# lionl1106/Clip-Neural-image-conpression

Hardware: AMD Instinct MI355X
Metric: images/sec @256px 50-step DDIM, batch=8/GPU (higher is better)
Workload: dtype bf16; 1 GPU; 256px base=128 ch_mult=(1, 2, 2) 50-step DDIM (eta=0), batch=8/GPU, key-seeded synthetic weights (out.* x0.1), synthetic z / x_T; global_batch=8, parallelism=dp1 (independent batches, no collective in the loop), graph=hipGraph, one replay per step, steps_in_flight=1

## Files before the change

clip-neural-image-conpression_amd/csrc/ccn_conv_pr.hip:

```cpp
#include "ccn_device.h"
#include <cstdio>
#include <cstdlib>
#include <cstring>
#include <vector>
#include <algorithm>

namespace ccn {

namespace {

#define CCN_FDIV(x, m, d) ((m) ? (int)__umulhi((unsigned)(x), (m)) : (int)(x))

template <int TH_> struct PrLdsT {
    static constexpr int HROWS = TH_ + 2, HPITCH = 34;
    static constexpr int A_BYTES = HROWS * HPITCH * 128;
    static constexpr int SP = 272;
    static constexpr int STG_BYTES = TH_ * 32 * SP;
    static constexpr int CHS_BYTES = 4 * 128 * 2 * 4;
    static constexpr int TOTAL = 2 * A_BYTES + STG_BYTES + CHS_BYTES;
};
typedef PrLdsT<8> PrLds;
static_assert(PrLds::TOTAL <= 160 * 1024, "LDS budget");

}

template <int NTAPS, int D, int MODE, int TH = 8, int GS = 0, bool P4 = false>
__global__ __launch_bounds__(512) void conv_pr_kernel(const ConvArgs a, const int grid_tiles)
{
    static_assert(TH == 8 || (TH == 4 && NTAPS == 9), "4-row tiles: 3x3 stride-1 form only");
    static_assert(!P4 || (NTAPS == 4 && MODE != 2), "plane passes of 2x2 taps: the 4-tap consumers, no split-K");
    constexpr bool RES = MODE == 1;
    constexpr bool RR = MODE != 0;
    typedef __bf16 T;
    constexpr int MF = 4, NF = 2;
    constexpr int BN = 128;
    constexpr int HROWS = TH + 2;
    constexpr int OSC = (NTAPS == 4 && !P4) ? 2 : 1, NPARC = (NTAPS == 4 && !P4) ? 4 : 1;
    constexpr int EPC = 8, CKE = 64;
    constexpr int NSTEP = NTAPS * 4;
    constexpr bool S2 = NTAPS == 2;
    constexpr int NPASS = S2 ? 5 : (P4 ? 4 : 1);
    constexpr int IS = (S2 || P4) ? 2 : 1;
    static_assert(NSTEP % D == 0, "the register ring must wrap at the chunk boundary");
    using L = PrLdsT<TH>;
    constexpr int HPITCH = L::HPITCH;
    extern __shared__ __attribute__((aligned(16))) unsigned char smem[];
    unsigned char* const stg = smem + 2 * L::A_BYTES;

    const int tid = threadIdx.x, lane = tid & 63, wave = tid >> 6;
    const int r = lane & 31, h = lane >> 5;

    const int grid = (int)gridDim.x;
    const int vb = (grid & 7) == 0 ? ((int)blockIdx.x & 7) * (grid >> 3) + ((int)blockIdx.x >> 3) : (int)blockIdx.x;
    const int ntiles = grid_tiles;
    const int my_tiles = (ntiles - vb + grid - 1) / grid;
    auto vt = [&](int ti) __attribute__((always_inline)) { return vb + ti * grid; };
    const int ks = (MODE == 2 && a.ksplit == 2) ? 2 : 1;
    const unsigned xcc_id = MODE == 2 ? (unsigned)__builtin_amdgcn_s_getreg((3 << 11) | 20) : 0u;
    const int nck = a.nchunk / ks;
    const int ktotal = my_tiles * nck;
    auto vt_tile = [&](int v) __attribute__((always_inline)) { return ks == 2 ? (v >> 1) : v; };
    auto vt_kh = [&](int v) __attribute__((always_inline)) { return ks == 2 ? (v & 1) : 0; };

    const unsigned char* const inb = (const unsigned char*)a.in;
    constexpr bool gstat = GS == 1;
    static_assert(GS != 1 || (NTAPS == 9 && MODE != 2), "in-kernel statistics: 3x3 stride-1 layers without split-K");
    const bool gn = NTAPS == 9 && GS != 2 && !CCN_DBG_BIT(a, 32);
    constexpr unsigned OOB = 0x7FFFFFF0u;
    auto raw_barrier = [&]() __attribute__((always_inline)) {
        asm volatile("s_waitcnt lgkmcnt(0)" ::: "memory");
        __builtin_amdgcn_s_barrier();
        asm volatile("" ::: "memory");
    };
    auto stamp = [&](int slot) __attribute__((always_inline)) {
        if (CCN_STAMPS_PTR(a) && lane == 0 && (wave == 0 || wave == 4))
            CCN_STAMPS_PTR(a)[((size_t)blockIdx.x * 2 + (wave == 0 ? 0 : 1)) * 8 + slot] = __builtin_amdgcn_s_memrealtime();
    };
    [[maybe_unused]] unsigned long long t_bar = 0, t_a = 0, t_b = 0, t_w = 0, t_r = 0;
    const unsigned long long t_begin = CCN_STAMPS_PTR(a) ? __builtin_amdgcn_s_memtime() : 0;
    auto timed_barrier = [&]() __attribute__((always_inline)) {
        if (CCN_STAMPS_PTR(a)) { const unsigned long long t0 = __builtin_amdgcn_s_memtime(); raw_barrier(); t_bar += __builtin_amdgcn_s_memtime() - t0; }
        else raw_barrier();
    };
    auto stamp_cycles = [&]() __attribute__((always_inline)) {
        if (CCN_STAMPS_PTR(a) && lane == 0 && (wave == 0 || wave == 4)) {
            unsigned long long* st = CCN_STAMPS_PTR(a) + ((size_t)blockIdx.x * 2 + (wave == 0 ? 0 : 1)) * 8;
            st[3] = t_bar; st[4] = __builtin_amdgcn_s_memtime() - t_begin; st[5] = t_a; st[6] = t_b; st[7] = t_r;
        }
    };
    stamp(0);

    const int etid = tid & 255, ew = wave & 3;
    const int o16 = etid & 15, pr = etid >> 4;
    unsigned char* const outb = (unsigned char*)a.out;
    const unsigned char* const resb = (const unsigned char*)a.res;
    const unsigned out_bytes = (unsigned)((size_t)a.B * a.Hout * a.Wout * a.Cout * sizeof(T));
    float* const chs = (float*)(stg + L::STG_BYTES) + ew * 256;
    constexpr int NQ = TH / 2;
    u32x4 rr[RR ? 2 : 1][4];
    f32x4 fb[2], fs[RES ? 1 : 2], ft[RES ? 1 : 2];
    int e_b = 0, e_ty = 0, e_tx = 0, e_nt = 0, e_par = 0, e_kh = 0, e_tile = 0;
    bool pd_on = false;
    int pd_b = 0, pd_slot = 0, pd_n0 = 0;
    unsigned char* const kpartb = (unsigned char*)a.kpart;
    unsigned e_base = 0;
    int e_rows = 0;
    unsigned e_m0 = OOB, e_m1 = OOB;
    auto item_off = [&](unsigned eb, int it) __attribute__((always_inline)) -> unsigned {
        const unsigned rmask = (it >> 1) < e_rows ? 0u : OOB;
        return (eb + (unsigned)(it >> 1) * (unsigned)(OSC * a.Wout * a.Cout * (int)sizeof(T)) + (unsigned)((it & 1) * 16) * (unsigned)(OSC * a.Cout * (int)sizeof(T)))
               | ((it & 1) ? e_m1 : e_m0) | rmask;
    };
    auto epi_setup = [&](int v) __attribute__((always_inline)) {
        const int tile = vt_tile(v);
        e_kh = vt_kh(v); e_tile = tile;
        const int t2 = CCN_FDIV(tile, a.fd_nt, a.n_nt);
        e_nt = tile - t2 * a.n_nt;
        e_par = t2 % NPARC;
        const int sp = t2 / NPARC;
        {
            const int row = CCN_FDIV(sp, a.fd_tx, a.n_tx);
            e_tx = sp - row * a.n_tx;
            e_b = CCN_FDIV(sp, a.fd_sp, a.n_tx * a.n_ty);
            e_ty = row - e_b * a.n_ty;
        }
        const int nb = e_nt * BN + o16 * 8;
        const bool nvalid = nb < a.Cout;
        e_base = (unsigned)(((e_b * a.Hout + e_ty * TH * OSC + (e_par >> 1)) * a.Wout + (e_tx * 32 + pr) * OSC + (e_par & 1)) * a.Cout + nb) * (unsigned)sizeof(T);
        e_rows = a.MH - e_ty * TH;
        e_m0 = (nvalid && e_tx * 32 + pr < a.MW) ? 0u : OOB;
        e_m1 = (nvalid && e_tx * 32 + pr + 16 < a.MW) ? 0u : OOB;
    };
    auto res_on = [&]() __attribute__((always_inline)) -> bool { return RES || (MODE == 2 && ks == 2 && e_kh == 1); };
    auto res_batch = [&](int q, u32x4* dst) __attribute__((always_inline)) {
        if constexpr (RR) {
            if (res_on()) {
                const auto srd = __builtin_amdgcn_make_buffer_rsrc((void*)((ks == 2 && e_kh == 1) ? kpartb : (resb ? resb : outb)), 0, out_bytes, 0x00020000);
                unsigned eb = e_base; asm volatile("" : "+v"(eb));
                if (ks == 2 && e_kh == 1) {
#pragma unroll
// ... 88 lines not shown
                if (live) {
#pragma unroll
                    for (int e = 0; e < 8; ++e) { s1[e] += x[e]; s2[e] = fmaf(x[e], x[e], s2[e]); }
                }
                asm volatile("" : "+v"(s1[0]), "+v"(s1[1]), "+v"(s1[2]), "+v"(s1[3]), "+v"(s1[4]), "+v"(s1[5]), "+v"(s1[6]), "+v"(s1[7]));
                asm volatile("" : "+v"(s2[0]), "+v"(s2[1]), "+v"(s2[2]), "+v"(s2[3]), "+v"(s2[4]), "+v"(s2[5]), "+v"(s2[6]), "+v"(s2[7]));
                __builtin_amdgcn_sched_barrier(0);
            }
            if constexpr (RR) { if (q + 2 < q1) res_batch(q + 2, rr[q & 1]); }
        }
        if (first) {
            asm volatile("s_waitcnt vmcnt(0)" ::: "memory");
            if (lane == 0) __hip_atomic_store(a.kflag + (size_t)e_tile * 4 + ew, xcc_id + 1u, __ATOMIC_RELAXED, __HIP_MEMORY_SCOPE_AGENT);
        }
        if (a.part && !first) {
#pragma unroll
            for (int s = 16; s < 64; s <<= 1)
#pragma unroll
                for (int e = 0; e < 8; ++e) { s1[e] += __shfl_xor(s1[e], s); s2[e] += __shfl_xor(s2[e], s); }
            if (lane < 16) {
#pragma unroll
                for (int e = 0; e < 8; ++e) { chs[(lane * 8 + e) * 2] = s1[e]; chs[(lane * 8 + e) * 2 + 1] = s2[e]; }
            }
            pd_on = true; pd_b = e_b; pd_n0 = e_nt * BN;
            pd_slot = ((e_ty * a.n_tx + e_tx) * NPARC + e_par) * a.n_nt + e_nt;
        }
    };
    auto combine = [&]() __attribute__((always_inline)) {
        if (!pd_on) return;
        pd_on = false;
        const float* const all = (const float*)(stg + L::STG_BYTES);
        const int n0 = pd_n0;
        if (n0 >= a.Cout) return;
        const int nend = min(n0 + BN, a.Cout);
        const int g1 = CCN_FDIV(nend - 1, a.fd_cpg, a.cpg);
        for (int g = CCN_FDIV(n0, a.fd_cpg, a.cpg) + ew; g <= g1; g += 4) {
            const int clo = max(g * a.cpg, n0), chi = min((g + 1) * a.cpg, nend);
            float t1 = 0.f, t2 = 0.f;
            const float* const wa = all + (lane >> 4) * 256;
            for (int c = clo + (lane & 15); c < chi; c += 16) {
                t1 += wa[(c - n0) * 2]; t2 += wa[(c - n0) * 2 + 1];
            }
#pragma unroll
            for (int m = 32; m >= 1; m >>= 1) { t1 += __shfl_xor(t1, m); t2 += __shfl_xor(t2, m); }
            if (lane == 0) part_store(a.part + (size_t)(pd_b * a.G + g) * a.nslot + pd_slot, t1, t2);
        }
    };

    const int ptid = tid & 255;
    const int ck = ptid & 7, pcol = ptid >> 3;
    const int xrow = pcol >> 1, xcol = 32 + (pcol & 1);
    const bool xthr = ptid < HROWS * 16;
    constexpr int AIT = HROWS + 1;
    u32x4 areg[AIT];
    GnCoef<T> gk;
    unsigned rowm = 0;
    bool colv = false, xv = false;
    int rq_ti = 0, rq_c = 0;
    GnCoef<T> gkn;
    int q_b = 0, q_iy0 = 0, q_ix0 = 0, q_c = 0;
    bool q_tv = false;
    float st_mean = 0.f, st_rstd = 1.f, qn_mean = 0.f, qn_rstd = 1.f;
    int st_b = -1;
    f32x4 qn_g[2], qn_bt[2];
    unsigned svmask = 0u;
    float2 sv[8];
    auto stats_issue = [&](int b) __attribute__((always_inline)) {
        const int g = lane >> 3, sub = lane & 7;
        const int cpg = a.gs_cpg, pnt = a.gs_nnt, nsp = a.gs_nsp;
        const int jlo = CCN_FDIV(g * cpg, a.fd_gsbn, a.gs_bn), jhi = CCN_FDIV((g + 1) * cpg - 1, a.fd_gsbn, a.gs_bn), nj = jhi - jlo + 1;
        const float2* const base = a.gs_part + (size_t)(b * 8 + g) * ((size_t)nsp * pnt) + jlo;
        int off[8];
        svmask = 0u;
#pragma unroll
        for (int u = 0; u < 8; ++u) {
            const int e = sub + 8 * u;
            const int jj = CCN_FDIV(e, a.fd_gsnsp, nsp), sp = e - jj * nsp;
            const bool ok = jj < nj;
            off[u] = ok ? sp * pnt + jj : 0;
            svmask |= ok ? (1u << u) : 0u;
        }
#pragma unroll
        for (int u = 0; u < 8; ++u) sv[u] = base[off[u]];
    };
    auto stats_reduce = [&]() __attribute__((always_inline)) {
        double s1 = 0.0, s2 = 0.0;
#pragma unroll
        for (int u = 0; u < 8; ++u) { const bool ok = (svmask >> u) & 1u; s1 += ok ? (double)sv[u].x : 0.0; s2 += ok ? (double)sv[u].y : 0.0; }
#pragma unroll
        for (int m = 1; m < 8; m <<= 1) { s1 += __shfl_xor(s1, m); s2 += __shfl_xor(s2, m); }
        const double mean = s1 * a.gs_inv_count;
        double var = s2 * a.gs_inv_count - mean * mean;
        if (var < 0.0) var = 0.0;
        st_mean = (float)mean;
        st_rstd = __builtin_amdgcn_rsqf((float)(var + 1e-5));
    };
    int q_cbs = 0; bool q_cv = false, q_cv_i = false;
    auto decode = [&]() __attribute__((always_inline)) -> bool {
        const int v = vt(rq_ti);
        if (rq_c == 0) {
            q_tv = rq_ti < my_tiles;
            const int tile = vt_tile(q_tv ? v : vt(0));
            const int sp = CCN_FDIV(tile, a.fd_ntp, a.n_nt * NPARC);
            const int row = CCN_FDIV(sp, a.fd_tx, a.n_tx);
            const int tx = sp - row * a.n_tx;
            q_b = CCN_FDIV(sp, a.fd_sp, a.n_tx * a.n_ty);
            const int ty = row - q_b * a.n_ty;
            q_iy0 = ty * TH - 1; q_ix0 = tx * 32 - 1;
        }
        q_c = vt_kh(v) * nck + rq_c;
        const int cb = (q_c / NPASS) * CKE + ck * EPC;
        q_cv = q_tv && cb < a.Cin;
        q_cbs = q_cv ? cb : 0;
        const bool fresh = gstat && rq_c == 0 && q_tv && q_b != st_b;
        if (++rq_c == nck) { rq_c = 0; ++rq_ti; }
        return fresh;
    };
    auto coef_loads = [&]() __attribute__((always_inline)) {
        if (gstat) {
            qn_g[0] = *(const f32x4*)(a.gs_gamma + q_cbs); qn_g[1] = *(const f32x4*)(a.gs_gamma + q_cbs + 4);
            qn_bt[0] = *(const f32x4*)(a.gs_beta + q_cbs); qn_bt[1] = *(const f32x4*)(a.gs_beta + q_cbs + 4);
        } else gkn.load(a.gn_ab + (size_t)q_b * a.Cin + q_cbs, gn && q_cv);
    };
    auto coef_sel = [&]() __attribute__((always_inline)) {
        if (gstat) {
            const int src = CCN_FDIV(q_cbs, a.fd_gscpg, a.gs_cpg) * 8;
            qn_mean = __shfl(st_mean, src); qn_rstd = __shfl(st_rstd, src);
        }
    };
    auto prep = [&]() __attribute__((always_inline)) {
        const bool fresh = decode();
        coef_loads();
        if (fresh) { stats_issue(q_b); stats_reduce(); st_b = q_b; }
        coef_sel();
    };
    auto adopt = [&]() __attribute__((always_inline)) {
        if (gstat) gk.from_raw(qn_g, qn_bt, qn_mean, qn_rstd, gn && q_cv_i);
        else gk = gkn;
    };
    auto issue_loads = [&](int r0 = 0, int r1 = TH + 2, bool with_x = true) __attribute__((always_inline)) {
        const int b = __builtin_amdgcn_readfirstlane(q_b), iy0 = __builtin_amdgcn_readfirstlane(q_iy0), ix0 = __builtin_amdgcn_readfirstlane(q_ix0);
        const int cc = __builtin_amdgcn_readfirstlane(q_c / NPASS);
        const int pass = q_c - cc * NPASS;
        const int py = S2 ? (pass <= 2 ? 1 : 0) : (P4 ? (pass < 2 ? 1 : 0) : 0);
        const int px = S2 ? ((pass <= 1 || pass == 3) ? 1 : 0) : (P4 ? ((pass & 1) ? 0 : 1) : 0);
        const int cb = cc * CKE + ck * EPC;
        const bool cv = q_tv && cb < a.Cin;
        q_cv_i = cv;
        const unsigned img_bytes = (unsigned)(a.Hin * a.Win * a.Cin) * (unsigned)sizeof(T);
        const unsigned coff = (unsigned)(((q_tv && cc * CKE < a.Cin) ? cc : 0) * CKE) * (unsigned)sizeof(T);
        const auto srd = __builtin_amdgcn_make_buffer_rsrc((void*)(inb + (size_t)b * img_bytes + coff), 0, img_bytes - coff, 0x00020000);
        const int rs = IS * a.Win * a.Cin * (int)sizeof(T);
        const int ixr = IS * (ix0 + pcol) + px;
        colv = cv && ixr >= 0 && ixr < a.Win;
        const unsigned cmask = colv ? 0u : OOB;
        const int base = ((IS * iy0 + py) * a.Win + ixr) * a.Cin * (int)sizeof(T) + ck * 16;
        const int first = IS * iy0 + py;
        const int r_lo = first < 0 ? (-first + IS - 1) / IS : 0;
        int r_hi = (a.Hin - first + IS - 1) / IS; r_hi = r_hi > HROWS ? HROWS : (r_hi < 0 ? 0 : r_hi);
        rowm = q_tv ? (((1u << r_hi) - 1u) & ~((1u << r_lo) - 1u)) : 0u;
#pragma unroll
        for (int i = 0; i < HROWS; ++i) {
            if (i < r0 || i >= r1) continue;
            areg[i] = __builtin_amdgcn_raw_buffer_load_b128(srd, (unsigned)(base + i * rs) | cmask, 0, 0);
        }
        {
            const int iyr = IS * (iy0 + xrow) + py, ixx = IS * (ix0 + xcol) + px;
            xv = xthr && cv && iyr >= 0 && iyr < a.Hin && ixx >= 0 && ixx < a.Win;
            const int off = (iyr * a.Win + ixx) * a.Cin * (int)sizeof(T) + ck * 16;
            if (with_x) areg[HROWS] = __builtin_amdgcn_raw_buffer_load_b128(srd, (unsigned)off | (xv ? 0u : OOB), 0, 0);
        }
    };
    auto issue = [&]() __attribute__((always_inline)) { issue_loads(); adopt(); };
    auto request = [&]() __attribute__((always_inline)) { prep(); issue(); };
    auto request_first = [&](int r0, int r1, bool with_x) __attribute__((always_inline)) {
        const bool fresh = decode();
        if (fresh) stats_issue(q_b);
        coef_loads();
        issue_loads(r0, r1, with_x);
        if (fresh) { stats_reduce(); st_b = q_b; }
        coef_sel();
        adopt();
    };
    auto dump = [&](int buf, int r0 = 0, int r1 = TH + 2, bool with_x = true) __attribute__((always_inline)) {
        unsigned char* const As = smem + buf * L::A_BYTES;
        int pc = pcol; asm volatile("" : "+v"(pc));
#pragma unroll
        for (int i = 0; i < AIT; ++i) {
            if (i < HROWS ? (i < r0 || i >= r1) : !with_x) continue;
            const int px = i < HROWS ? i * HPITCH + pc : (pc >> 1) * HPITCH + 32 + (pc & 1);
            const int sw = i < HROWS ? (NTAPS == 9 ? (pc >> 1) & 3 : (pc >> 1)) : 0;
            u32x4 v = areg[i];
            const bool ok = i < HROWS ? (((rowm >> i) & 1u) && colv) : xv;
            if (gn) {
                const u32x4 tr = gk.template apply<true>(v);
                v = u32x4{0u, 0u, 0u, 0u};
                if (ok) v = tr;
            }
            if (i < HROWS || xthr) *(u32x4*)(As + px * 128 + (((ck ^ sw) & 7) << 4)) = v;
            if ((i & 1) == 1) __builtin_amdgcn_sched_barrier(0);
        }
    };

    constexpr int HSPLIT = HROWS / 2;

    if (wave >= 4) {
        if (a.prod_first) __builtin_amdgcn_s_setprio(3);
        if (CCN_DBG_BIT(a, 128)) __builtin_amdgcn_s_setprio(1);
        if (CCN_DBG_BIT(a, 256)) __builtin_amdgcn_s_setprio(3);
        request_first(0, HSPLIT, true);
        dump(0, 0, HSPLIT, true);
        request();
        raw_barrier();
        stamp(1);
        int c = 0, ti = 0;
        for (int k = 0; k < ktotal; ++k) {
            unsigned long long t0 = CCN_STAMPS_PTR(a) ? __builtin_amdgcn_s_memtime() : 0;
            if (CCN_STAMPS_PTR(a)) {
                asm volatile("s_waitcnt vmcnt(0)" ::: "memory");
                const unsigned long long t1 = __builtin_amdgcn_s_memtime(); t_w += t1 - t0; t0 = t1;
            }
            if (k + 1 < ktotal) { prep(); dump((k + 1) & 1); }
            if (CCN_STAMPS_PTR(a)) { const unsigned long long t1 = __builtin_amdgcn_s_memtime(); t_a += t1 - t0; t0 = t1; }
            const bool epi = c == 0 && ti > 0;
            if (epi) epi_request(0, NQ);
            if (k + 1 < ktotal) issue();
            if (c == nck - 1) epi_setup(vt(ti));
            if (CCN_STAMPS_PTR(a)) { const unsigned long long t1 = __builtin_amdgcn_s_memtime(); t_r += t1 - t0; t0 = t1; }
            if (epi) epilogue(0, NQ);
            if (CCN_STAMPS_PTR(a)) t_b += __builtin_amdgcn_s_memtime() - t0;
            const bool early = k + 1 == ktotal && !(ks == 2 && e_kh == 1);
            if (early) epi_request(0, NQ);
            timed_barrier();
            combine();
            if (++c == nck) { c = 0; ++ti; }
        }
        if (ks == 2 && e_kh == 1) epi_request(0, NQ);
        epilogue(0, NQ);
        if (pd_on) {
            raw_barrier();
            combine();
        }
        stamp(2); stamp_cycles();
        return;
    }

    if (!CCN_DBG_BIT(a, 16)) __builtin_amdgcn_s_setprio(2);
    if constexpr (NTAPS == 9) {
        constexpr int NROW = HROWS, NSG = 2 * NROW;
        constexpr int NG = 6;
        constexpr int WIN = 6, PF = 4;
        static_assert((NG * NSG) % WIN == 0, "static window indexing");
        f32x16 acc[TH];
        const int n32 = a.Cout_pad / 32;
        constexpr unsigned COLB = 36 * 1024;
        const unsigned wtotal = (unsigned)((size_t)a.nchunk * n32 * COLB);
        const auto wsrd = __builtin_amdgcn_make_buffer_rsrc((void*)a.wfrag, 0, wtotal, 0x00020000);
        const unsigned lane16 = (unsigned)lane * 16u;
        auto wbase_of = [&](int tile, int chunk) __attribute__((always_inline)) -> unsigned {
            const int nt = tile - CCN_FDIV(tile, a.fd_nt, a.n_nt) * a.n_nt;
            return (unsigned)__builtin_amdgcn_readfirstlane((int)((unsigned)(chunk * n32 + nt * 4 + wave) * COLB));
        };
        const int px16 = lane & 15, g4 = lane >> 4;
        int b16x[3];
#pragma unroll
        for (int d = 0; d < 3; ++d) { const int hx = px16 + d; b16x[d] = hx * 128 + ((((g4 & 1) << 2) | ((g4 >> 1) ^ ((hx >> 1) & 3))) << 4); }
        u32x4 bq[2][3][2];
        {
            const unsigned wb = wbase_of(vt_tile(vt(0)), vt_kh(vt(0)) * nck);
#pragma unroll
            for (int f = 0; f < 6; ++f) bq[0][f >> 1][f & 1] = __builtin_amdgcn_raw_buffer_load_b128(wsrd, lane16, wb + f * 1024, 0);
        }
        const int stg_lane = px16 * L::SP + (wave * 32 + 4 * g4) * 2;
        if constexpr (HSPLIT < HROWS) {
            request_first(HSPLIT, HROWS, false);
            if (CCN_STAMPS_PTR(a)) {
                const unsigned long long r0 = CCN_STAMPS_PTR(a)[((size_t)blockIdx.x * 2) * 8];
                t_a = __builtin_amdgcn_s_memrealtime() - r0;
                asm volatile("s_waitcnt vmcnt(0)" ::: "memory");
                t_b = __builtin_amdgcn_s_memrealtime() - r0;
            }
            dump(0, HSPLIT, HROWS, false);
            if (CCN_STAMPS_PTR(a)) t_r = __builtin_amdgcn_s_memrealtime() - CCN_STAMPS_PTR(a)[((size_t)blockIdx.x * 2) * 8];
        }
        raw_barrier();
        stamp(1);
        int k = 0;
        const bool idle_w = ks == 1 && grid % a.n_nt == 0 &&
                            (vt_tile(vt(0)) - CCN_FDIV(vt_tile(vt(0)), a.fd_nt, a.n_nt) * a.n_nt) * BN + wave * 32 >= a.Cout;
        if (idle_w) { for (int kk = 0; kk < ktotal; ++kk) timed_barrier(); }
        else
        for (int ti = 0; ti < my_tiles; ++ti) {
            const int v = vt(ti), v_next = ti + 1 < my_tiles ? vt(ti + 1) : v;
            const int tile = vt_tile(v), c0 = vt_kh(v) * nck;
#pragma unroll
            for (int i = 0; i < TH; ++i)
#pragma unroll
                for (int q = 0; q < 16; ++q) acc[i][q] = 0.0f;
            for (int chunk = 0; chunk < nck; ++chunk, ++k) {
                const unsigned wb_cur = wbase_of(tile, c0 + chunk);
                const unsigned wb_nxt = chunk + 1 < nck ? wbase_of(tile, c0 + chunk + 1) : wbase_of(vt_tile(v_next), vt_kh(v_next) * nck);
                int bufoff = (k & 1) * L::A_BYTES; asm volatile("" : "+v"(bufoff));
                u32x4 rw[WIN];
                int ag = 0;
                auto rload = [&](int s_) __attribute__((always_inline)) {
                    const int g = s_ / NSG, hp = s_ % NSG;
                    if (hp == 0) ag = (bufoff + b16x[g >> 1]) ^ ((g & 1) << 5);
                    rw[s_ % WIN] = *(const u32x4*)(smem + ag + ((hp >> 1) * HPITCH + (hp & 1) * 16) * 128);
                };
                if (!CCN_DBG_BIT(a, 64)) {
#pragma unroll
                for (int s_ = 0; s_ < PF; ++s_) rload(s_);
#pragma unroll
                for (int s_ = 0; s_ < NG * NSG; ++s_) {
                    const int g = s_ / NSG, hh = (s_ % NSG) >> 1, p = s_ & 1;
                    __builtin_amdgcn_sched_barrier(0);
                    const bool wl = TH == 8 ? (p == 0 && hh >= 2 && hh <= 7) : (hh >= 1 && hh <= 3);
                    if (wl) {
                        const int f = TH == 8 ? hh - 2 : (hh - 1) * 2 + p;
                        const unsigned off = g + 1 < NG ? wb_cur + (unsigned)((g + 1) * 6 + f) * 1024u : wb_nxt + (unsigned)f * 1024u;
                        bq[(g + 1) & 1][f >> 1][f & 1] = __builtin_amdgcn_raw_buffer_load_b128(wsrd, lane16, off, 0);
                    }
                    if (s_ + PF < NG * NSG) rload(s_ + PF);
                    int nm = 0;
#pragma unroll
                    for (int q6 = 0; q6 < 6; ++q6) {
                        const int o = (s_ & 1) ? 5 - q6 : q6;
                        const int dy = o >> 1, c = o & 1;
                        const int i = hh - dy;
                        if (i >= 0 && i < TH) { mfma16q(acc[i], p * 2 + c, bq[g & 1][dy][c], rw[s_ % WIN]); ++nm; }
                    }
#pragma unroll
                    for (int m = 0; m < 6; ++m) {
                        if (m < nm) __builtin_amdgcn_sched_group_barrier(0x008, 1, 0);
                        if (m == 0) __builtin_amdgcn_sched_group_barrier(0x100, 1, 0);
                        if (m == 2 && wl) __builtin_amdgcn_sched_group_barrier(0x020, 1, 0);
// ... 156 lines not shown
    }
    if (gs == 2 && ntaps == 9) {
        if (th == 4) return mode == 1 ? (pr_fn_t)conv_pr_kernel<9, PR_D, 1, 4, 2> : (mode == 2 ? (pr_fn_t)conv_pr_kernel<9, PR_D, 2, 4, 2> : (pr_fn_t)conv_pr_kernel<9, PR_D, 0, 4, 2>);
        return mode == 1 ? (pr_fn_t)conv_pr_kernel<9, PR_D, 1, 8, 2> : (mode == 2 ? (pr_fn_t)conv_pr_kernel<9, PR_D, 2, 8, 2> : (pr_fn_t)conv_pr_kernel<9, PR_D, 0, 8, 2>);
    }
    if (ntaps == 9 && th == 4) return mode == 1 ? (pr_fn_t)conv_pr_kernel<9, PR_D, 1, 4> : (mode == 2 ? (pr_fn_t)conv_pr_kernel<9, PR_D, 2, 4> : (pr_fn_t)conv_pr_kernel<9, PR_D, 0, 4>);
    if (ntaps == 9) return mode == 1 ? (pr_fn_t)conv_pr_kernel<9, PR_D, 1> : (mode == 2 ? (pr_fn_t)conv_pr_kernel<9, PR_D, 2> : (pr_fn_t)conv_pr_kernel<9, PR_D, 0>);
    if (ntaps == 2) return mode == 1 ? (pr_fn_t)conv_pr_kernel<2, 8, 1> : (mode == 2 ? (pr_fn_t)conv_pr_kernel<2, 8, 2> : (pr_fn_t)conv_pr_kernel<2, 8, 0>);
    return mode == 1 ? (pr_fn_t)conv_pr_kernel<4, 8, 1> : (mode == 2 ? (pr_fn_t)conv_pr_kernel<4, 8, 2> : (pr_fn_t)conv_pr_kernel<4, 8, 0>);
}

bool conv_pr_supported(int kind, int bn, int th)
{
    return bn == 128 && (((kind == KIND_C3S1 || kind == KIND_CT4 || kind == KIND_C3S2) && th == 8) || (kind == KIND_C3S1 && th == 4));
}

static int g_cus = 0;
hipError_t conv_pr_prepare()
{
    hipError_t e = hipSuccess;
    for (int ntaps : {2, 4, 9, 16})
        for (int mode = 0; mode < 3; ++mode) {
            if (ntaps == 16 && mode == 2) continue;
            e = hipFuncSetAttribute((const void*)pick_pr(ntaps, mode), hipFuncAttributeMaxDynamicSharedMemorySize, (int)PrLds::TOTAL);
            if (e != hipSuccess) return e;
        }
    for (int mode = 0; mode < 3; ++mode) {
        e = hipFuncSetAttribute((const void*)pick_pr(9, mode, 4), hipFuncAttributeMaxDynamicSharedMemorySize, (int)PrLdsT<4>::TOTAL);
        if (e != hipSuccess) return e;
    }
    for (int gs = 1; gs <= 2; ++gs)
        for (int mode = 0; mode < 3; ++mode) {
            if (gs == 1 && mode == 2) continue;
            e = hipFuncSetAttribute((const void*)pick_pr(9, mode, 8, gs), hipFuncAttributeMaxDynamicSharedMemorySize, (int)PrLds::TOTAL);
            if (e != hipSuccess) return e;
            e = hipFuncSetAttribute((const void*)pick_pr(9, mode, 4, gs), hipFuncAttributeMaxDynamicSharedMemorySize, (int)PrLdsT<4>::TOTAL);
            if (e != hipSuccess) return e;
        }
    int dev = 0;
    e = hipGetDevice(&dev);
    if (e != hipSuccess) return e;
    hipDeviceProp_t prop;
    e = hipGetDeviceProperties(&prop, dev);
    if (e != hipSuccess) return e;
    g_cus = prop.multiProcessorCount;
    return hipSuccess;
}

static unsigned long long* g_stamps = nullptr;
static unsigned g_stamp_grid = 0;
extern "C" int ccn_internal_dump_stamps_pr(const char* path)
{
    if (!g_stamps || !g_stamp_grid) return 1;
    std::vector<unsigned long long> hbuf((size_t)g_stamp_grid * 16);
    if (hipMemcpy(hbuf.data(), g_stamps, hbuf.size() * 8, hipMemcpyDeviceToHost) != hipSuccess) return 2;
    FILE* f = fopen(path, "w");
    if (!f) return 3;
    for (unsigned b = 0; b < g_stamp_grid; ++b)
        for (int k = 0; k < 16; ++k) fprintf(f, "%llu%c", hbuf[(size_t)b * 16 + k], k == 15 ? '\n' : ' ');
    fclose(f);
    return 0;
}

hipError_t launch_conv_pr(int dtype, const ConvArgs& a, hipStream_t s)
{
    const bool c3 = a.ntaps == 9 && a.npar == 1 && a.OS == 1, ct = a.ntaps == 4 && a.npar == 4 && a.OS == 2;
    const bool s2 = a.ntaps == 2 && a.npar == 1 && a.OS == 1 && !a.gn_ab && (a.nchunk % 5) == 0;
    const bool p4 = a.ntaps == 16 && a.npar == 1 && a.OS == 1 && (a.nchunk % 4) == 0 && a.ksplit != 2;
    if ((ct || s2 || p4) && (a.gn_ab || a.gs_part)) return hipErrorInvalidValue;
    if (dtype != 1 || !a.wfrag || !(c3 || ct || s2 || p4) || !(a.th == 8 || (a.th == 4 && c3)) || (a.Cout_pad & 127) || a.nchunk < 2 || a.fin_counter || (a.res && a.film)) return hipErrorInvalidValue;
    const int ks = a.ksplit == 2 ? 2 : 1;
    if (ks == 2 && (!a.kpart || !a.kflag || (a.nchunk & 1) || (s2 && (a.nchunk / 2) % 5) || a.res)) return hipErrorInvalidValue;
    const int ntiles = a.B * a.n_ty * a.n_tx * a.npar * a.n_nt * ks;
    static const int cap = diag_env("CCN_PR_GRID") ? atoi(diag_env("CCN_PR_GRID")) : 0;
    int grid = cap > 0 ? cap : (g_cus > 0 ? g_cus : 256);
    if (grid > ntiles) grid = ntiles;
    if (ks == 2) { grid &= ~15; if (grid < 16) return hipErrorInvalidValue; }
    ConvArgs d = a;
    {
        auto magic = [](long dv) -> unsigned { return dv <= 1 ? 0u : (unsigned)((0x100000000ull + (unsigned long long)dv - 1) / (unsigned long long)dv); };
        const long dmax = std::max<long>(std::max<long>((long)a.n_nt * a.npar, (long)a.n_tx * a.n_ty), std::max<long>(a.cpg, a.gs_cpg));
        if ((unsigned long long)std::max<long>(ntiles, 8192) * (unsigned long long)dmax >= 0x100000000ull) return hipErrorInvalidValue;
        d.fd_nt = magic(a.n_nt); d.fd_ntp = magic((long)a.n_nt * a.npar); d.fd_tx = magic(a.n_tx); d.fd_sp = magic((long)a.n_tx * a.n_ty);
        d.fd_cpg = magic(a.cpg); d.fd_gscpg = magic(a.gs_cpg);
        d.fd_gsbn = magic(a.gs_bn); d.fd_gsnsp = magic(a.gs_nsp);
    }
    d.prod_first = (a.nchunk <= 2 && c3) ? 1 : 0;
    static const char* env = diag_env("CCN_STAMPS");
    if (env && (unsigned)atoi(env) == (unsigned)ntiles && (!strchr(env, ':') || atoi(strchr(env, ':') + 1) == a.ntaps)) {
        if (!g_stamps) { if (hipMalloc((void**)&g_stamps, (size_t)1024 * 24 * 8) != hipSuccess) return hipErrorOutOfMemory; }
        g_stamp_grid = (unsigned)grid;
        d.stamps = g_stamps;
    } else d.stamps = nullptr;
    if (a.gs_part && !(c3 && ks == 1)) return hipErrorInvalidValue;
    hipLaunchKernelGGL(pick_pr(a.ntaps, a.res ? 1 : (ks == 2 ? 2 : 0), a.th, a.gs_part ? 1 : (a.gn_ab ? 0 : 2)), dim3((unsigned)grid), dim3(512),
                       a.th == 4 ? PrLdsT<4>::TOTAL : PrLds::TOTAL, s, d, ntiles);
    return hipGetLastError();
}

}
```

clip-neural-image-conpression_amd/csrc/ccn_kernels.hip:

```cpp
#include "ccn_conv_tile.h"

namespace ccn {

__host__ __device__ constexpr int cmax(int a, int b) { return a > b ? a : b; }

template <int AK, int IS> struct HaloGeom {
    static constexpr int HOFF = AK == A_NHWC ? 1 : 0;
    static constexpr int ROWS = AK == A_NHWC ? (IS == 1 ? 6 : 10) : 4;
    static constexpr int PITCH = AK == A_NHWC ? (IS == 1 ? 34 : 66) : 32;
    static constexpr int BYTES = ROWS * PITCH * 128;
};
template <int AK, int IS, int BN> struct LdsGeom {
    static constexpr int A_BYTES = HaloGeom<AK, IS>::BYTES;
    static constexpr int B_BYTES = BN * 128;
    static constexpr int TOTAL = EpiLds<4, BN, 4>::total(A_BYTES + 2 * B_BYTES);
};

template <typename T, int AK, int IS, int EPI, int WM, int WN, int MF, int NF>
__global__ __launch_bounds__(256) void conv_igemm_kernel(const ConvArgs a)
{
    static_assert(WM * WN == 4 && WM * MF == 4, "4 waves, 4 M-fragments of 32 pixels (TH=4 rows of TW=32)");
    constexpr int BN = WN * NF * 32;
    constexpr int EPC = Vec16<T>::EPC;
    constexpr int CKE = 8 * EPC;
// ... 632 lines not shown
    const int per = (HW + nslot - 1) / nslot;
    const int p0 = slot * per, p1 = min(HW, p0 + per);
    const int nsub = 256 / G;
    const int g = tid % G, sub = tid / G;
    float s1 = 0.f, s2 = 0.f;
    if (sub < nsub)
        for (int p = p0 + sub; p < p1; p += nsub) {
            const T* row = x + ((size_t)b * HW + p) * C + g * cpg;
            for (int j = 0; j < cpg; ++j) { const float v = (float)row[j]; s1 += v; s2 = fmaf(v, v, s2); }
        }
    sh[tid * 2] = s1; sh[tid * 2 + 1] = s2;
    __syncthreads();
    if (tid < G) {
        float t1 = 0.f, t2 = 0.f;
        for (int q = 0; q < nsub; ++q) { t1 += sh[(q * G + tid) * 2]; t2 += sh[(q * G + tid) * 2 + 1]; }
        part[(size_t)(b * G + tid) * nslot + slot] = make_float2(t1, t2);
    }
}
hipError_t launch_gn_partials(int dtype, const void* x, float2* part, int B, int HW, int C, int cpg, int G, int nslot, hipStream_t s)
{
    if (G > 256) return hipErrorInvalidValue;
    if (dtype == 0) hipLaunchKernelGGL(gn_partials_kernel<float>, dim3(nslot, B), dim3(256), 0, s, (const float*)x, part, HW, C, cpg, G, nslot);
    else hipLaunchKernelGGL(gn_partials_kernel<__bf16>, dim3(nslot, B), dim3(256), 0, s, (const __bf16*)x, part, HW, C, cpg, G, nslot);
    return hipGetLastError();
}

template <typename TI>
__global__ void temb_kernel(const TI* __restrict__ t, float* __restrict__ out, int n, int dim)
{
    const int half = dim / 2;
    const int idx = blockIdx.x * blockDim.x + threadIdx.x;
    if (idx >= n * dim) return;
    const int row = idx / dim, i = idx - row * dim;
    float v = 0.0f;
    if (i < 2 * half) {
        const int fi = i < half ? i : i - half;
        const float f = expf(__fdiv_rn(__fmul_rn(-9.210340371976184f, (float)fi), (float)half));
        const float arg = __fmul_rn((float)t[row], f);
        v = i < half ? cosf(arg) : sinf(arg);
    }
    out[idx] = v;
}
hipError_t launch_temb_i64(const int64_t* t, float* out, int n, int dim, hipStream_t s)
{
    hipLaunchKernelGGL(temb_kernel<int64_t>, dim3((n * dim + 255) / 256), dim3(256), 0, s, t, out, n, dim);
    return hipGetLastError();
}
hipError_t launch_temb_i32(const int32_t* t, float* out, int n, int dim, hipStream_t s)
{
    hipLaunchKernelGGL(temb_kernel<int32_t>, dim3((n * dim + 255) / 256), dim3(256), 0, s, t, out, n, dim);
    return hipGetLastError();
}

__global__ __launch_bounds__(256) void linear_kernel(const float* __restrict__ xa, const float* __restrict__ xb, int a_div, int b_mod,
                                                      const float* __restrict__ W, const float* __restrict__ bias, float* __restrict__ y,
                                                      int R, int K, int N, int act_silu)
{
    const int lane = threadIdx.x & 63, wave = threadIdx.x >> 6;
    const int n = blockIdx.x * 4 + wave;
    if (n >= N) return;
    const int r0 = blockIdx.y * 16, r1 = min(R, r0 + 16);
    const float* wrow = W + (size_t)n * K;
    for (int rr = r0; rr < r1; ++rr) {
        const float* pa = xa + (size_t)(rr / a_div) * K;
        const float* pb = xb ? xb + (size_t)(rr % b_mod) * K : nullptr;
        float acc = 0.f;
        for (int k = lane; k < K; k += 64) {
            float xv = pa[k];
            if (pb) xv += pb[k];
            acc = fmaf(xv, wrow[k], acc);
        }
#pragma unroll
        for (int s = 32; s >= 1; s >>= 1) acc += __shfl_xor(acc, s);
        if (lane == 0) {
            float v = acc + (bias ? bias[n] : 0.f);
            if (act_silu) v = v / (1.0f + expf(-v));
            y[(size_t)rr * N + n] = v;
        }
    }
}
hipError_t launch_linear(const float* xa, const float* xb, int a_div, int b_mod, const float* W, const float* b, float* y,
                         int R, int K, int N, int act_silu, hipStream_t s)
{
    hipLaunchKernelGGL(linear_kernel, dim3((N + 3) / 4, (R + 15) / 16), dim3(256), 0, s, xa, xb, a_div, b_mod, W, b, y, R, K, N, act_silu);
    return hipGetLastError();
}

__global__ void ddim_step_kernel(float* __restrict__ x, const float* __restrict__ eps, const float* __restrict__ noise,
                                 float c0, float c1, float c2, float c3, float sigma, int64_t n)
{
    for (int64_t i = (int64_t)blockIdx.x * blockDim.x + threadIdx.x; i < n; i += (int64_t)gridDim.x * blockDim.x) {
        const float e = eps[i];
        float x0 = __fdiv_rn(__fsub_rn(x[i], __fmul_rn(c0, e)), c1);
        x0 = fminf(fmaxf(x0, -1.0f), 1.0f);
        float xn = __fadd_rn(__fmul_rn(c2, x0), __fmul_rn(c3, e));
        if (noise) xn = __fadd_rn(xn, __fmul_rn(sigma, noise[i]));
        x[i] = xn;
    }
}
hipError_t launch_ddim_step(float* x, const float* eps, const float* noise, float c0, float c1, float c2, float c3, float sigma,
                            int64_t n, hipStream_t s)
{
    const int grid = (int)((n + 255) / 256 < 4096 ? (n + 255) / 256 : 4096);
    hipLaunchKernelGGL(ddim_step_kernel, dim3(grid > 0 ? grid : 1), dim3(256), 0, s, x, eps, noise, c0, c1, c2, c3, sigma, n);
    return hipGetLastError();
}

__global__ void q_sample_kernel(float* __restrict__ out, const float* __restrict__ x0, const float* __restrict__ noise,
                                const float* __restrict__ a, const float* __restrict__ sg, int64_t per)
{
    const int b = blockIdx.y;
    const float ca = a[b], cs = sg[b];
    const size_t base = (size_t)b * per;
    for (int64_t i = (int64_t)blockIdx.x * blockDim.x + threadIdx.x; i < per; i += (int64_t)gridDim.x * blockDim.x)
        out[base + i] = __fadd_rn(__fmul_rn(ca, x0[base + i]), __fmul_rn(cs, noise[base + i]));
}
hipError_t launch_q_sample(float* out, const float* x0, const float* noise, const float* a, const float* sg, int B, int64_t per,
                           hipStream_t s)
{
    const int gx = (int)((per + 255) / 256 < 1024 ? (per + 255) / 256 : 1024);
    hipLaunchKernelGGL(q_sample_kernel, dim3(gx > 0 ? gx : 1, B), dim3(256), 0, s, out, x0, noise, a, sg, per);
    return hipGetLastError();
}

__global__ void predict_x0_kernel(float* __restrict__ out, const float* __restrict__ xt, const float* __restrict__ eps,
                                  const float* __restrict__ a, const float* __restrict__ sg, int64_t per)
{
    const int b = blockIdx.y;
    const float ca = a[b], cs = sg[b];
    const size_t base = (size_t)b * per;
    for (int64_t i = (int64_t)blockIdx.x * blockDim.x + threadIdx.x; i < per; i += (int64_t)gridDim.x * blockDim.x)
        out[base + i] = __fdiv_rn(__fsub_rn(xt[base + i], __fmul_rn(cs, eps[base + i])), ca);
}
hipError_t launch_predict_x0(float* out, const float* xt, const float* eps, const float* a, const float* sg, int B, int64_t per,
                             hipStream_t s)
{
    const int gx = (int)((per + 255) / 256 < 1024 ? (per + 255) / 256 : 1024);
// ... 58 lines not shown
```

Before: 83.83 images/sec.

## Double-buffer plane-pass register loads and register-tile the linear kernel

For the 2- and 4-tap conv forms, the register staging ring gets two sets so that loads for chunk k+2 are in flight while chunk k+1 is dumped to LDS. This hides global load latency at the cost of more VGPRs. Separately, the small linear kernel now keeps the weight row in registers, processes four rows per batch with interleaved shuffles, and covers 32 rows per block. The stamp instrumentation is widened to record the extra counters.

Result: no change. 83.33 images/sec (-0.6%).

```diff
diff --git a/clip-neural-image-conpression_amd/csrc/ccn_conv_pr.hip b/clip-neural-image-conpression_amd/csrc/ccn_conv_pr.hip
--- a/clip-neural-image-conpression_amd/csrc/ccn_conv_pr.hip
+++ b/clip-neural-image-conpression_amd/csrc/ccn_conv_pr.hip
@@ -4,12 +4,17 @@
 #include <cstring>
 #include <vector>
 #include <algorithm>
+#include <type_traits>
 
 namespace ccn {
 
 namespace {
 
 #define CCN_FDIV(x, m, d) ((m) ? (int)__umulhi((unsigned)(x), (m)) : (int)(x))
+
+#ifndef CCN_PR_PLANE_DEPTH
+#define CCN_PR_PLANE_DEPTH 2
+#endif
 
 template <int TH_> struct PrLdsT {
     static constexpr int HROWS = TH_ + 2, HPITCH = 34;
@@ -42,6 +47,7 @@
     constexpr int NPASS = S2 ? 5 : (P4 ? 4 : 1);
     constexpr int IS = (S2 || P4) ? 2 : 1;
     static_assert(NSTEP % D == 0, "the register ring must wrap at the chunk boundary");
+    constexpr int DEPTH = (CCN_PR_PLANE_DEPTH == 2 && (NTAPS == 2 || NTAPS == 4)) ? 2 : 1;
     using L = PrLdsT<TH>;
     constexpr int HPITCH = L::HPITCH;
     extern __shared__ __attribute__((aligned(16))) unsigned char smem[];
@@ -74,7 +80,7 @@
     };
     auto stamp = [&](int slot) __attribute__((always_inline)) {
         if (CCN_STAMPS_PTR(a) && lane == 0 && (wave == 0 || wave == 4))
-            CCN_STAMPS_PTR(a)[((size_t)blockIdx.x * 2 + (wave == 0 ? 0 : 1)) * 8 + slot] = __builtin_amdgcn_s_memrealtime();
+            CCN_STAMPS_PTR(a)[((size_t)blockIdx.x * 3 + (wave == 0 ? 0 : 1)) * 8 + slot] = __builtin_amdgcn_s_memrealtime();
     };
     [[maybe_unused]] unsigned long long t_bar = 0, t_a = 0, t_b = 0, t_w = 0, t_r = 0;
     const unsigned long long t_begin = CCN_STAMPS_PTR(a) ? __builtin_amdgcn_s_memtime() : 0;
@@ -84,8 +90,14 @@
     };
     auto stamp_cycles = [&]() __attribute__((always_inline)) {
         if (CCN_STAMPS_PTR(a) && lane == 0 && (wave == 0 || wave == 4)) {
-            unsigned long long* st = CCN_STAMPS_PTR(a) + ((size_t)blockIdx.x * 2 + (wave == 0 ? 0 : 1)) * 8;
+            unsigned long long* st = CCN_STAMPS_PTR(a) + ((size_t)blockIdx.x * 3 + (wave == 0 ? 0 : 1)) * 8;
             st[3] = t_bar; st[4] = __builtin_amdgcn_s_memtime() - t_begin; st[5] = t_a; st[6] = t_b; st[7] = t_r;
+            if (wave == 4) {
+                unsigned long long* sx = CCN_STAMPS_PTR(a) + ((size_t)blockIdx.x * 3 + 2) * 8;
+                sx[0] = t_w; sx[1] = (unsigned long long)ktotal; sx[2] = (unsigned long long)DEPTH;
+#pragma unroll
+                for (int i = 3; i < 8; ++i) sx[i] = 0;
+            }
         }
     };
     stamp(0);
@@ -280,10 +292,10 @@
     const int xrow = pcol >> 1, xcol = 32 + (pcol & 1);
     const bool xthr = ptid < HROWS * 16;
     constexpr int AIT = HROWS + 1;
-    u32x4 areg[AIT];
+    u32x4 areg[DEPTH][AIT];
     GnCoef<T> gk;
-    unsigned rowm = 0;
-    bool colv = false, xv = false;
+    unsigned rowm[DEPTH] = {};
+    bool colv[DEPTH] = {}, xv[DEPTH] = {};
     int rq_ti = 0, rq_c = 0;
     GnCoef<T> gkn;
     int q_b = 0, q_iy0 = 0, q_ix0 = 0, q_c = 0;
@@ -366,7 +378,7 @@
         if (gstat) gk.from_raw(qn_g, qn_bt, qn_mean, qn_rstd, gn && q_cv_i);
         else gk = gkn;
     };
-    auto issue_loads = [&](int r0 = 0, int r1 = TH + 2, bool with_x = true) __attribute__((always_inline)) {
+    auto issue_loads = [&](int r0 = 0, int r1 = TH + 2, bool with_x = true, int set = 0) __attribute__((always_inline)) {
         const int b = __builtin_amdgcn_readfirstlane(q_b), iy0 = __builtin_amdgcn_readfirstlane(q_iy0), ix0 = __builtin_amdgcn_readfirstlane(q_ix0);
         const int cc = __builtin_amdgcn_readfirstlane(q_c / NPASS);
         const int pass = q_c - cc * NPASS;
@@ -380,27 +392,28 @@
         const auto srd = __builtin_amdgcn_make_buffer_rsrc((void*)(inb + (size_t)b * img_bytes + coff), 0, img_bytes - coff, 0x00020000);
         const int rs = IS * a.Win * a.Cin * (int)sizeof(T);
         const int ixr = IS * (ix0 + pcol) + px;
-        colv = cv && ixr >= 0 && ixr < a.Win;
-        const unsigned cmask = colv ? 0u : OOB;
+        colv[set] = cv && ixr >= 0 && ixr < a.Win;
+        const unsigned cmask = colv[set] ? 0u : OOB;
         const int base = ((IS * iy0 + py) * a.Win + ixr) * a.Cin * (int)sizeof(T) + ck * 16;
         const int first = IS * iy0 + py;
         const int r_lo = first < 0 ? (-first + IS - 1) / IS : 0;
         int r_hi = (a.Hin - first + IS - 1) / IS; r_hi = r_hi > HROWS ? HROWS : (r_hi < 0 ? 0 : r_hi);
-        rowm = q_tv ? (((1u << r_hi) - 1u) & ~((1u << r_lo) - 1u)) : 0u;
+        rowm[set] = q_tv ? (((1u << r_hi) - 1u) & ~((1u << r_lo) - 1u)) : 0u;
 #pragma unroll
         for (int i = 0; i < HROWS; ++i) {
             if (i < r0 || i >= r1) continue;
-            areg[i] = __builtin_amdgcn_raw_buffer_load_b128(srd, (unsigned)(base + i * rs) | cmask, 0, 0);
+            areg[set][i] = __builtin_amdgcn_raw_buffer_load_b128(srd, (unsigned)(base + i * rs) | cmask, 0, 0);
         }
         {
             const int iyr = IS * (iy0 + xrow) + py, ixx = IS * (ix0 + xcol) + px;
-            xv = xthr && cv && iyr >= 0 && iyr < a.Hin && ixx >= 0 && ixx < a.Win;
+            xv[set] = xthr && cv && iyr >= 0 && iyr < a.Hin && ixx >= 0 && ixx < a.Win;
             const int off = (iyr * a.Win + ixx) * a.Cin * (int)sizeof(T) + ck * 16;
-            if (with_x) areg[HROWS] = __builtin_amdgcn_raw_buffer_load_b128(srd, (unsigned)off | (xv ? 0u : OOB), 0, 0);
+            if (with_x) areg[set][HROWS] = __builtin_amdgcn_raw_buffer_load_b128(srd, (unsigned)off | (xv[set] ? 0u : OOB), 0, 0);
         }
     };
     auto issue = [&]() __attribute__((always_inline)) { issue_loads(); adopt(); };
     auto request = [&]() __attribute__((always_inline)) { prep(); issue(); };
+    auto request_set = [&](int set) __attribute__((always_inline)) { prep(); issue_loads(0, TH + 2, true, set); adopt(); };
     auto request_first = [&](int r0, int r1, bool with_x) __attribute__((always_inline)) {
         const bool fresh = decode();
         if (fresh) stats_issue(q_b);
@@ -410,7 +423,7 @@
         coef_sel();
         adopt();
     };
-    auto dump = [&](int buf, int r0 = 0, int r1 = TH + 2, bool with_x = true) __attribute__((always_inline)) {
+    auto dump = [&](int buf, int r0 = 0, int r1 = TH + 2, bool with_x = true, int set = 0) __attribute__((always_inline)) {
         unsigned char* const As = smem + buf * L::A_BYTES;
         int pc = pcol; asm volatile("" : "+v"(pc));
 #pragma unroll
@@ -418,8 +431,8 @@
             if (i < HROWS ? (i < r0 || i >= r1) : !with_x) continue;
             const int px = i < HROWS ? i * HPITCH + pc : (pc >> 1) * HPITCH + 32 + (pc & 1);
             const int sw = i < HROWS ? (NTAPS == 9 ? (pc >> 1) & 3 : (pc >> 1)) : 0;
-            u32x4 v = areg[i];
-            const bool ok = i < HROWS ? (((rowm >> i) & 1u) && colv) : xv;
+            u32x4 v = areg[set][i];
+            const bool ok = i < HROWS ? (((rowm[set] >> i) & 1u) && colv[set]) : xv[set];
             if (gn) {
                 const u32x4 tr = gk.template apply<true>(v);
                 v = u32x4{0u, 0u, 0u, 0u};
@@ -438,10 +451,50 @@
         if (CCN_DBG_BIT(a, 256)) __builtin_amdgcn_s_setprio(3);
         request_first(0, HSPLIT, true);
         dump(0, 0, HSPLIT, true);
-        request();
+        if constexpr (DEPTH == 2) {
+            request_set(1);
+            __builtin_amdgcn_sched_barrier(0);
+            request_set(0);
+        } else request();
         raw_barrier();
         stamp(1);
         int c = 0, ti = 0;
+        if constexpr (DEPTH == 2) {
+            auto iter2 = [&](const int k, auto set_c) __attribute__((always_inline)) {
+                constexpr int set = decltype(set_c)::value;
+                unsigned long long t0 = CCN_STAMPS_PTR(a) ? __builtin_amdgcn_s_memtime() : 0;
+                if (CCN_STAMPS_PTR(a)) {
+                    asm volatile("s_waitcnt vmcnt(%0)" :: "n"(AIT) : "memory");
+                    const unsigned long long t1 = __builtin_amdgcn_s_memtime(); t_w += t1 - t0; t0 = t1;
+                }
+                if (set == 1 || k + 1 < ktotal) dump((k + 1) & 1, 0, TH + 2, true, set);
+                if (CCN_STAMPS_PTR(a)) { const unsigned long long t1 = __builtin_amdgcn_s_memtime(); t_a += t1 - t0; t0 = t1; }
+                const bool epi = c == 0 && ti > 0;
+                if (epi) epi_request(0, NQ);
+                if (c == nck - 1) epi_setup(vt(ti));
+                if (CCN_STAMPS_PTR(a)) { const unsigned long long t1 = __builtin_amdgcn_s_memtime(); t_r += t1 - t0; t0 = t1; }
+                if (epi) epilogue(0, NQ);
+                if (CCN_STAMPS_PTR(a)) { const unsigned long long t1 = __builtin_amdgcn_s_memtime(); t_b += t1 - t0; t0 = t1; }
+                const bool early = set == 0 && k + 1 == ktotal && !(ks == 2 && e_kh == 1);
+                if (early) epi_request(0, NQ);
+                request_set(set);
+                if (CCN_STAMPS_PTR(a)) t_r += __builtin_amdgcn_s_memtime() - t0;
+                timed_barrier();
+                combine();
+                if (++c == nck) { c = 0; ++ti; }
+            };
+            int k = 0;
+            for (; k + 2 <= ktotal; k += 2) {
+                iter2(k, std::integral_constant<int, 1>{});
+                iter2(k + 1, std::integral_constant<int, 0>{});
+            }
+            if (k < ktotal) {
+                epi_setup(vt(ti));
+                if (!(ks == 2 && e_kh == 1)) epi_request(0, NQ);
+                timed_barrier();
+                combine();
+            }
+        } else
         for (int k = 0; k < ktotal; ++k) {
             unsigned long long t0 = CCN_STAMPS_PTR(a) ? __builtin_amdgcn_s_memtime() : 0;
             if (CCN_STAMPS_PTR(a)) {
@@ -503,13 +556,13 @@
         if constexpr (HSPLIT < HROWS) {
             request_first(HSPLIT, HROWS, false);
             if (CCN_STAMPS_PTR(a)) {
-                const unsigned long long r0 = CCN_STAMPS_PTR(a)[((size_t)blockIdx.x * 2) * 8];
+                const unsigned long long r0 = CCN_STAMPS_PTR(a)[((size_t)blockIdx.x * 3) * 8];
                 t_a = __builtin_amdgcn_s_memrealtime() - r0;
                 asm volatile("s_waitcnt vmcnt(0)" ::: "memory");
                 t_b = __builtin_amdgcn_s_memrealtime() - r0;
             }
             dump(0, HSPLIT, HROWS, false);
-            if (CCN_STAMPS_PTR(a)) t_r = __builtin_amdgcn_s_memrealtime() - CCN_STAMPS_PTR(a)[((size_t)blockIdx.x * 2) * 8];
+            if (CCN_STAMPS_PTR(a)) t_r = __builtin_amdgcn_s_memrealtime() - CCN_STAMPS_PTR(a)[((size_t)blockIdx.x * 3) * 8];
         }
         raw_barrier();
         stamp(1);
@@ -772,12 +825,12 @@
 extern "C" int ccn_internal_dump_stamps_pr(const char* path)
 {
     if (!g_stamps || !g_stamp_grid) return 1;
-    std::vector<unsigned long long> hbuf((size_t)g_stamp_grid * 16);
+    std::vector<unsigned long long> hbuf((size_t)g_stamp_grid * 24);
     if (hipMemcpy(hbuf.data(), g_stamps, hbuf.size() * 8, hipMemcpyDeviceToHost) != hipSuccess) return 2;
     FILE* f = fopen(path, "w");
     if (!f) return 3;
     for (unsigned b = 0; b < g_stamp_grid; ++b)
-        for (int k = 0; k < 16; ++k) fprintf(f, "%llu%c", hbuf[(size_t)b * 16 + k], k == 15 ? '\n' : ' ');
+        for (int k = 0; k < 24; ++k) fprintf(f, "%llu%c", hbuf[(size_t)b * 24 + k], k == 23 ? '\n' : ' ');
     fclose(f);
     return 0;
 }
@@ -807,7 +860,9 @@
     }
     d.prod_first = (a.nchunk <= 2 && c3) ? 1 : 0;
     static const char* env = diag_env("CCN_STAMPS");
-    if (env && (unsigned)atoi(env) == (unsigned)ntiles && (!strchr(env, ':') || atoi(strchr(env, ':') + 1) == a.ntaps)) {
+    const char* const env2 = env ? strchr(env, ':') : nullptr;
+    const char* const env3 = env2 ? strchr(env2 + 1, ':') : nullptr;
+    if (env && (unsigned)atoi(env) == (unsigned)ntiles && (!env2 || atoi(env2 + 1) == a.ntaps) && (!env3 || atoi(env3 + 1) == a.Cin)) {
         if (!g_stamps) { if (hipMalloc((void**)&g_stamps, (size_t)1024 * 24 * 8) != hipSuccess) return hipErrorOutOfMemory; }
         g_stamp_grid = (unsigned)grid;
         d.stamps = g_stamps;
diff --git a/clip-neural-image-conpression_amd/csrc/ccn_kernels.hip b/clip-neural-image-conpression_amd/csrc/ccn_kernels.hip
--- a/clip-neural-image-conpression_amd/csrc/ccn_kernels.hip
+++ b/clip-neural-image-conpression_amd/csrc/ccn_kernels.hip
@@ -708,6 +708,8 @@
     return hipGetLastError();
 }
 
+constexpr int LIN_ROWS = 32, LIN_RB = 4;
+template <int KR>
 __global__ __launch_bounds__(256) void linear_kernel(const float* __restrict__ xa, const float* __restrict__ xb, int a_div, int b_mod,
                                                       const float* __restrict__ W, const float* __restrict__ bias, float* __restrict__ y,
                                                       int R, int K, int N, int act_silu)
@@ -715,30 +717,72 @@
     const int lane = threadIdx.x & 63, wave = threadIdx.x >> 6;
     const int n = blockIdx.x * 4 + wave;
     if (n >= N) return;
-    const int r0 = blockIdx.y * 16, r1 = min(R, r0 + 16);
+    const int r0 = blockIdx.y * LIN_ROWS, r1 = min(R, r0 + LIN_ROWS);
     const float* wrow = W + (size_t)n * K;
-    for (int rr = r0; rr < r1; ++rr) {
-        const float* pa = xa + (size_t)(rr / a_div) * K;
-        const float* pb = xb ? xb + (size_t)(rr % b_mod) * K : nullptr;
-        float acc = 0.f;
-        for (int k = lane; k < K; k += 64) {
-            float xv = pa[k];
-            if (pb) xv += pb[k];
-            acc = fmaf(xv, wrow[k], acc);
-        }
-#pragma unroll
-        for (int s = 32; s >= 1; s >>= 1) acc += __shfl_xor(acc, s);
+    const float bn = bias ? bias[n] : 0.f;
+    auto finish = [&](float acc, int rr) __attribute__((always_inline)) {
         if (lane == 0) {
-            float v = acc + (bias ? bias[n] : 0.f);
+            float v = acc + bn;
             if (act_silu) v = v / (1.0f + expf(-v));
             y[(size_t)rr * N + n] = v;
         }
+    };
+    if constexpr (KR == 0) {
+        for (int rr = r0; rr < r1; ++rr) {
+            const float* pa = xa + (size_t)(rr / a_div) * K;
+            const float* pb = xb ? xb + (size_t)(rr % b_mod) * K : nullptr;
+            float acc = 0.f;
+            for (int k = lane; k < K; k += 64) {
+                float xv = pa[k];
+                if (pb) xv += pb[k];
+                acc = fmaf(xv, wrow[k], acc);
+            }
+#pragma unroll
+            for (int s = 32; s >= 1; s >>= 1) acc += __shfl_xor(acc, s);
+            finish(acc, rr);
+        }
+    } else {
+        float w[KR];
+#pragma unroll
+        for (int j = 0; j < KR; ++j) w[j] = lane + 64 * j < K ? wrow[lane + 64 * j] : 0.f;
+        for (int rb = r0; rb < r1; rb += LIN_RB) {
+            float xv[LIN_RB][KR], acc[LIN_RB];
+#pragma unroll
+            for (int i = 0; i < LIN_RB; ++i) {
+                const int rr = min(rb + i, r1 - 1);
+                const float* pa = xa + (size_t)(rr / a_div) * K;
+#pragma unroll
+                for (int j = 0; j < KR; ++j) xv[i][j] = lane + 64 * j < K ? pa[lane + 64 * j] : 0.f;
+            }
+            if (xb) {
+#pragma unroll
+                for (int i = 0; i < LIN_RB; ++i) {
+                    const int rr = min(rb + i, r1 - 1);
+                    const float* pb = xb + (size_t)(rr % b_mod) * K;
+#pragma unroll
+                    for (int j = 0; j < KR; ++j) { if (lane + 64 * j < K) xv[i][j] += pb[lane + 64 * j]; }
+                }
+            }
+#pragma unroll
+            for (int i = 0; i < LIN_RB; ++i) {
+                acc[i] = 0.f;
+#pragma unroll
+                for (int j = 0; j < KR; ++j) { if (lane + 64 * j < K) acc[i] = fmaf(xv[i][j], w[j], acc[i]); }
+            }
+#pragma unroll
+            for (int s = 32; s >= 1; s >>= 1)
+#pragma unroll
+                for (int i = 0; i < LIN_RB; ++i) acc[i] += __shfl_xor(acc[i], s);
+#pragma unroll
+            for (int i = 0; i < LIN_RB; ++i) { if (rb + i < r1) finish(acc[i], rb + i); }
+        }
     }
 }
 hipError_t launch_linear(const float* xa, const float* xb, int a_div, int b_mod, const float* W, const float* b, float* y,
                          int R, int K, int N, int act_silu, hipStream_t s)
 {
-    hipLaunchKernelGGL(linear_kernel, dim3((N + 3) / 4, (R + 15) / 16), dim3(256), 0, s, xa, xb, a_div, b_mod, W, b, y, R, K, N, act_silu);
+    const auto fn = K <= 256 ? linear_kernel<4> : (K <= 512 ? linear_kernel<8> : (K <= 1024 ? linear_kernel<16> : linear_kernel<0>));
+    hipLaunchKernelGGL(fn, dim3((N + 3) / 4, (R + LIN_ROWS - 1) / LIN_ROWS), dim3(256), 0, s, xa, xb, a_div, b_mod, W, b, y, R, K, N, act_silu);
     return hipGetLastError();
 }
 
```
